# 2noise/ChatTTS

Measured on NVIDIA H100. Metric: speech-tokens/sec (GPT decode loop, 4-codebook tokens; RTF = wall / audio seconds @ 24 kHz), higher is better.
Workload: dtype f32

## Files before the change

### chattts_b200/csrc/flow.cuh

```cuda
#pragma once
#include "gpt_kernels.cuh"
#include "tc_common.cuh"

namespace ctb {

constexpr int FL_THREADS = 256;
constexpr int FL_LAUNCH_THREADS = FL_THREADS;
constexpr int FL_WARPS = 8;
constexpr int FL_SLOTS = 4;
constexpr int FL_SLOT_BYTES = 6144;
constexpr int FL_SLOT_FLOATS = FL_SLOT_BYTES / 4;
constexpr int FL_RING_BYTES = FL_WARPS * FL_SLOTS * FL_SLOT_BYTES;
constexpr int FL_SMAX = 6;
constexpr int FL_CH = 64;
constexpr int FL_PW = 66;
constexpr int FL_BMAX = 4;
constexpr int FL_ROWS = 6;
constexpr int FL_GU = 3;
constexpr int FL_QR = 2;
constexpr int FL_HEADS = 12;
constexpr int FL_RMAX = 16;

constexpr int FL_A_X = 0;
constexpr int FL_A_XO = FL_A_X + FL_BMAX * KC;
constexpr int FL_A_ACT = FL_A_XO + FL_BMAX * KC;
constexpr int FL_A_P = FL_A_ACT + FL_BMAX * 4 * KC;
constexpr int FL_A_END = FL_A_P + FL_BMAX * FL_HEADS * FL_SMAX * FL_PW;
constexpr int FL_REP_STRIDE = ((FL_A_END + 1023) / 1024) * 1024;
constexpr int FL_A_Q = 0, FL_A_KN = FL_BMAX * KC, FL_A_VN = 2 * FL_BMAX * KC;
constexpr int FL_QKV_WORDS = 3 * FL_BMAX * KC;
constexpr int FL_SROWS = 16, FL_VPAD = 1024;
constexpr int FL_A_LOGITS = FL_QKV_WORDS, FL_A_IDX = FL_A_LOGITS + FL_SROWS * FL_VPAD;
constexpr int FL_TAIL_WORDS = FL_A_IDX + 64;
constexpr size_t FL_PARITY_WORDS = (size_t)FL_RMAX * FL_REP_STRIDE + FL_TAIL_WORDS;
constexpr size_t FL_ARENA_WORDS = 2 * FL_PARITY_WORDS;
constexpr unsigned FL_EPOCH_STEP = 256;
constexpr int FL_TR_EV = 4096, FL_TR_EVN = 32, FL_TR_WORDS = FL_TR_EV + 192 * FL_TR_EVN;

enum FlowTagKind { FT_X = 0, FT_QKV = 1, FT_P = 2, FT_XO = 3, FT_ACT = 4, FT_LOGITS = 5, FT_IDX = 6 };
enum FlowStage { FS_Q0 = 0, FS_Q1 = 1, FS_KV = 2, FS_O = 3, FS_GU0 = 4, FS_GU1 = 5, FS_GU2 = 6, FS_D0 = 7, FS_D1 = 8, FS_NLAYER = 9 };

__device__ __forceinline__ void fl_bar() { asm volatile("bar.sync 1, 256;" ::: "memory"); }

struct FlowP {
  const float* W;
  int64_t layer0, layer_stride, o_wqkv, o_wo, o_wgu, o_wd, o_ln1, o_ln2, o_final_norm, o_head, o_emb_code, o_emb_text,
      o_cos, o_sin;
  int L, I, Hq, hd;
  float eps, scaling;
  float *logits, *kv;
  size_t kv_layer_floats;
  const int* block_table; int pages_per_row;
  int* seq_len;
  LoopState* st;
  int decode, col, T0, sample;
  const float* emb; const uint8_t* mask; const int32_t* ids_out;
  int max_new, num_vq, num_audio, infer_text, B;
  float* hidden_out; int hidden_stride, rows_per_item, V;
  unsigned long long* arena;
  unsigned* epoch;
  int R;
  int l2_ahead;
  unsigned long long* trace;
  int nsteps;
  int ink;
  ctb_sampler_config samp;
  const float* q_noise;
  uint8_t* finish;
  int* end_idx;
  int32_t* ids_w;
};

__device__ __forceinline__ void ll_st(unsigned long long* p, float v, uint32_t tag) {
  const unsigned long long x = ((unsigned long long)tag << 32) | (unsigned long long)__float_as_uint(v);
  asm volatile("st.relaxed.gpu.global.u64 [%0], %1;" ::"l"(p), "l"(x) : "memory");
}
__device__ __forceinline__ unsigned long long ll_ld(const unsigned long long* p) {
  unsigned long long x;
  asm volatile("ld.global.cg.u64 %0, [%1];" : "=l"(x) : "l"(p) : "memory");
  return x;
}
__device__ __forceinline__ void ll_ld2(const unsigned long long* p, unsigned long long& a, unsigned long long& b) {
  asm volatile("ld.global.cg.v2.u64 {%0,%1}, [%2];" : "=l"(a), "=l"(b) : "l"(p) : "memory");
}
__device__ __forceinline__ uint32_t ll_tag(unsigned long long x) { return (uint32_t)(x >> 32); }
__device__ __forceinline__ float ll_val(unsigned long long x) { return __uint_as_float((uint32_t)x); }

struct FlowWd {
  int* err;
  int dead;
  int spins;
};
__device__ __forceinline__ bool fl_giveup(FlowWd& wd, int code) {
  if (wd.dead) return true;
  if (++wd.spins < (1 << 20)) {
// ... 118 lines not shown
      const int bytes = e.z & 0xffff, ncopy = (e.z >> 16) & 0xf, kind = e.z >> 20;
      const float* src = (kind ? p.kv + (size_t)it.l * p.kv_layer_floats : p.W + p.layer0 + (int64_t)it.l * p.layer_stride) + e.x;
      fl_expect(bar, (uint32_t)(bytes * ncopy));
#pragma unroll
      for (int k = 0; k < 4; ++k)
        if (k < ncopy) fl_bulk(dst + k * bytes, src + (int64_t)k * e.y, (uint32_t)bytes, bar, kind ? pol_kv : pol_w);
      if (p.l2_ahead && kind == 0) {
        const float* nsrc = it.l + 1 < p.L ? src + p.layer_stride : src - (int64_t)(p.L - 1) * p.layer_stride;
#pragma unroll
        for (int k = 0; k < 4; ++k)
          if (k < ncopy)
            asm volatile("cp.async.bulk.prefetch.L2.global [%0], %1;" ::"l"(nsrc + (int64_t)k * e.y), "r"((uint32_t)bytes) : "memory");
      }
    }
    if (++it.k == it.ntab) { it.k = 0; it.l++; }
    it.n++;
    return true;
  }
  if (gs->cta * FL_WARPS + w + it.hsub * gs->NW < gs->nheads_tasks) {
    fl_issue_heads(p, gs, w, it.hsub, dst, bar, pol_w);
    it.hsub++;
    it.n++;
    return true;
  }
  return false;
}

struct FlowW {
  float* base;
  uint32_t ring;
  uint32_t bars;
  int n;
  int owed;
  FlowIss it;
  const int4* tab;
  const FlowGeo* gs;
  uint64_t pol_w, pol_kv;
};
__device__ __forceinline__ void fl_refill(const FlowP& p, FlowW& w) {
  if (w.owed > 0) {
    __syncwarp();
    fl_issue(p, w.gs, w.tab, w.it, (int)(threadIdx.x >> 5), w.ring, w.bars, w.pol_w, w.pol_kv);
    w.owed--;
  }
}
__device__ __forceinline__ const float* fl_ring_slot_at(const FlowW& w, int k) { return w.base + ((w.n + k) % FL_SLOTS) * FL_SLOT_FLOATS; }
__device__ __forceinline__ bool fl_ring_peek_n(const FlowP& p, FlowW& w, int cnt) {
  while (w.owed > FL_SLOTS - cnt) fl_refill(p, w);
  bool ok = true;
#pragma unroll
  for (int k = 0; k < 3; ++k)
    if (k < cnt) { const int n = w.n + k; ok = fl_try_wait(w.bars + (n % FL_SLOTS) * 8, (uint32_t)(n / FL_SLOTS) & 1u) && ok; }
  return ok;
}
__device__ __forceinline__ void fl_ring_wait_n(const FlowP& p, FlowW& w, int cnt, FlowWd& wd) {
  while (w.owed > FL_SLOTS - cnt) fl_refill(p, w);
  uint32_t bar[3], par[3];
#pragma unroll
  for (int k = 0; k < 3; ++k) {
    const int n = w.n + k;
    bar[k] = w.bars + (n % FL_SLOTS) * 8;
    par[k] = (uint32_t)(n / FL_SLOTS) & 1u;
  }
  wd.spins = 0;
  while (true) {
    bool ok[3];
#pragma unroll
    for (int k = 0; k < 3; ++k) ok[k] = k < cnt ? fl_try_wait(bar[k], par[k]) : true;
    if (ok[0] && ok[1] && ok[2]) break;
    if (__any_sync(0xffffffffu, fl_giveup(wd, 0x120))) { wd.dead = 1; break; }
  }
}
__device__ __forceinline__ const float* fl_ring_wait(const FlowP& p, FlowW& w, FlowWd& wd) {
  fl_ring_wait_n(p, w, 1, wd);
  return fl_ring_slot_at(w, 0);
}
__device__ __forceinline__ void fl_ring_release(const FlowP& p, FlowW& w) { w.n++; w.owed++; fl_refill(p, w); }
__device__ __forceinline__ void fl_refill_all(const FlowP& p, FlowW& w) {
  while (w.owed > 0) fl_refill(p, w);
}

template <int BT>
__device__ __forceinline__ void fl_stage768(const FlowP& p, const unsigned long long* src, uint32_t tag, float* xs, FlowWd& wd, FlowW& fw) {
  const int tid = threadIdx.x;
  unsigned long long v[BT][3];
  wd.spins = 0;
  while (true) {
    bool ok = true;
#pragma unroll
    for (int b = 0; b < BT; ++b)
      if (b < p.B) {
#pragma unroll
        for (int k = 0; k < 3; ++k) v[b][k] = ll_ld(src + b * KC + tid + 256 * k);
      }
#pragma unroll
    for (int b = 0; b < BT; ++b)
      if (b < p.B) {
#pragma unroll
        for (int k = 0; k < 3; ++k) ok = ok && (ll_tag(v[b][k]) == tag);
      }
    if (__all_sync(0xffffffffu, ok)) break;
    if (__any_sync(0xffffffffu, fl_giveup(wd, 0x200 + (tag & 0xff)))) { wd.dead = 1; break; }
  }
#pragma unroll
  for (int b = 0; b < BT; ++b) {
#pragma unroll
    for (int k = 0; k < 3; ++k) xs[b * KC + tid + 256 * k] = b < p.B ? ll_val(v[b][k]) : 0.f;
  }
  fl_bar();
}

template <int BT>
// ... 425 lines not shown
  __shared__ __align__(8) uint64_t s_nwbar[2];
  __shared__ int s_pos[BT], s_active[BT], s_page[BT];
  __shared__ float s_cos[BT * 64], s_sin[BT * 64];
  __shared__ float s_red[FL_ROWS][FL_WARPS][BT];
  __shared__ float s_resd[FL_ROWS * BT];
  __shared__ float s_am[FL_WARPS], s_al[FL_WARPS];
  __shared__ __align__(16) float s_ao[FL_WARPS][64];
  __shared__ FlowGeo s_geo;
  __shared__ __align__(16) float s_nw1[KC], s_nw2[KC];
  __shared__ int4 s_tab[FL_WARPS][FL_TMAX];
  __shared__ FlowSamp s_samp_store[BT <= 2 ? 1 : 0 + (BT > 2)];
  FlowSamp& s_samp = s_samp_store[0];

  const int tid = threadIdx.x, lane = tid & 31, warp = tid >> 5;
  constexpr int LPB = 32 / BT;
  if (tid < FL_WARPS * FL_SLOTS) mbar_init(&s_bar[tid], 1);
  if (tid < 2) mbar_init(&s_nwbar[tid], 1);
  asm volatile("fence.mbarrier_init.release.cluster;" ::: "memory");
  __syncthreads();
  pdl_trigger();
  pdl_wait();
  if (p.decode && ldg_cg(&p.st->all_finished)) return;

  constexpr bool INK = BT <= 2;
  __shared__ int s_ids[BT * 8];
  __shared__ int s_fin[BT], s_end[BT];
  __shared__ int s_allfin;
  FlowWd wd{&p.st->err, 0, 0};
  uint32_t base = (uint32_t)ldg_cg(reinterpret_cast<const int*>(p.epoch));
  int tr = 0;
#define FL_TRACE() do { if (p.trace && blockIdx.x == 0 && tid == 0 && tr < 250) p.trace[tr++] = globaltimer_ns(); } while (0)
#define FL_EV(k) do { if (p.trace && l == 10 && tid == 0) p.trace[FL_TR_EV + blockIdx.x * FL_TR_EVN + (k)] = globaltimer_ns(); } while (0)
#define FL_CK(k) do { if (p.trace && l == 10 && tid == 0 && blockIdx.x == 0) p.trace[3000 + (k)] = (unsigned long long)clock64(); } while (0)

  int ngen = p.decode ? ldg_cg(&p.st->n_gen) : 0;
  int lstep = p.decode ? ldg_cg(&p.st->step) : 0;
  if (tid < BT) {
    int act = 0, pos = 0;
    if (tid < p.B) {
      pos = ldg_cg(&p.seq_len[tid]);
      act = p.decode ? 1 : (p.mask[(size_t)tid * p.T0 + p.col] != 0);
    }
    s_pos[tid] = pos; s_active[tid] = act;
    s_fin[tid] = (tid < p.B && p.ink) ? (int)p.finish[tid] : 0;
    s_end[tid] = (tid < p.B && p.ink) ? ldg_cg(&p.end_idx[tid]) : 0;
  }
  const bool ink = INK && p.ink != 0;
  const int nrows_s = p.B * p.rows_per_item;
  const int R = p.R;
  uint64_t pol_w, pol_kv;
  asm volatile("createpolicy.fractional.L2::evict_first.b64 %0, 1.0;" : "=l"(pol_w));
  asm volatile("createpolicy.fractional.L2::evict_normal.b64 %0, 1.0;" : "=l"(pol_kv));
  int nw1_cnt = 0, nw2_cnt = 0;
  FlowW fw;
  fw.base = reinterpret_cast<float*>(fl_smem) + (size_t)warp * FL_SLOTS * FL_SLOT_FLOATS;
  fw.ring = smem_u32(fw.base);
  fw.bars = smem_u32(&s_bar[warp * FL_SLOTS]);
  fw.n = 0; fw.owed = 0;
  fw.it = FlowIss{0, 0, 0, 0, 0};
  fw.tab = s_tab[warp]; fw.gs = &s_geo; fw.pol_w = pol_w; fw.pol_kv = pol_kv;
  FlowGeo g;
  g.G = gridDim.x; g.NW = g.G * FL_WARPS; g.cta = blockIdx.x; g.warp = warp; g.lane = lane; g.gw = g.cta * FL_WARPS + warp;
  g.S = max(1, min(FL_SMAX, g.G / (p.Hq * p.B)));
  g.nheads_tasks = p.sample ? (p.rows_per_item * p.V + 1) / 2 : 0;
  const int myrep = g.cta % R;
  const int o_row = g.cta + g.G * warp;
  unsigned long long* tailw = p.arena + (size_t)FL_RMAX * FL_REP_STRIDE;
  fl_bar();

  int nwin = 0;
  if constexpr (INK) {
    if (ink && g.cta < nrows_s) {
      const int item = g.cta / p.rows_per_item, qi = g.cta % p.rows_per_item;
      const bool pen = p.samp.penalty_on && g.cta < p.samp.penalty_max_ids;
      nwin = pen ? min(ngen, p.samp.past_window) : 0;
      if (tid < nwin) s_samp.win[tid] = ldg_cg(&p.ids_out[((size_t)item * p.max_new + (ngen - nwin + tid)) * p.num_vq + qi]);
    }
  }

#define FL_PREP_STEP()                                                                                                  \
  do {                                                                                                                  \
    if (tid < BT) s_page[tid] = tid < p.B ? __ldg(p.block_table + tid * p.pages_per_row + s_pos[tid] / kPageTokens) : 0; \
    {                                                                                                                   \
      const int u = g.cta;                                                                                              \
      g.u_on = 0; g.u_b = 0; g.u_h = 0; g.u_split = 0; g.u_n = 0; g.u_nchunk = 0;                                       \
      if (u < p.B * p.Hq * g.S) {                                                                                       \
        g.u_split = u % g.S; g.u_h = (u / g.S) % p.Hq; g.u_b = u / (g.S * p.Hq);                                        \
        g.u_n = s_pos[g.u_b] + 1;                                                                                       \
        g.u_nchunk = (g.u_n + FL_CH - 1) / FL_CH;                                                                       \
        g.u_on = s_active[g.u_b] && g.u_split < min(g.u_nchunk, g.S);                                                   \
      }                                                                                                                 \
    }                                                                                                                   \
    if (tid == 0) s_geo = g;                                                                                            \
    fl_bar();                                                                                                           \
    fw.it.l = 0; fw.it.k = 0; fw.it.hsub = 0; fw.owed = 0;                                                              \
    fw.it.ntab = fl_build_table(p, &s_geo, s_tab[warp]);                                                                \
    __syncwarp();                                                                                                       \
    for (int k_ = 0; k_ < FL_SLOTS; ++k_) fl_issue(p, fw.gs, fw.tab, fw.it, warp, fw.ring, fw.bars, pol_w, pol_kv);     \
    for (int i = tid; i < BT * 64; i += FL_THREADS) {                                                                   \
      const int b = i / 64;                                                                                             \
      s_cos[i] = b < p.B ? __ldg(p.W + p.o_cos + (size_t)s_pos[b] * 64 + (i % 64)) : 0.f;                               \
      s_sin[i] = b < p.B ? __ldg(p.W + p.o_sin + (size_t)s_pos[b] * 64 + (i % 64)) : 0.f;                               \
    }                                                                                                                   \
  } while (0)

  FL_PREP_STEP();
  FL_TRACE();
#pragma unroll 1
  for (int sidx = 0;; ++sidx) {
  FL_TRACE();
  fl_nw_fetch(s_nw1, p.W + p.layer0 + p.o_ln1, &s_nwbar[0], pol_w);
  fl_nw_fetch(s_nw2, p.W + p.layer0 + p.o_ln2, &s_nwbar[1], pol_w);
  {
    float ev[BT * 3][8];
#pragma unroll
    for (int it_ = 0; it_ < BT * 3; ++it_) {
      const int i = tid + it_ * FL_THREADS, b = i / KC, k = i % KC;
#pragma unroll
      for (int q = 0; q < 8; ++q) ev[it_][q] = 0.f;
      if (b < p.B) {
        if (!p.decode) {
          ev[it_][0] = s_active[b] ? p.emb[((size_t)b * p.T0 + p.col) * KC + k] : 0.f;
        } else if (p.infer_text) {
          const int id0 = ldg_cg(p.ids_out + ((size_t)b * p.max_new + (ngen - 1)) * p.num_vq);
          ev[it_][0] = p.W[p.o_emb_text + (size_t)id0 * KC + k];
        } else {
#pragma unroll
          for (int q = 0; q < 8; ++q)
            if (q < p.num_vq) {
              const int id = sidx > 0 ? s_ids[b * 8 + q] : ldg_cg(p.ids_out + ((size_t)b * p.max_new + (ngen - 1)) * p.num_vq + q);
              ev[it_][q] = p.W[p.o_emb_code + ((size_t)q * p.num_audio + id) * KC + k];
            }
        }
      }
    }
#pragma unroll
    for (int it_ = 0; it_ < BT * 3; ++it_) {
      float v = 0.f;
#pragma unroll
      for (int q = 0; q < 8; ++q) v += ev[it_][q];
      xs[tid + it_ * FL_THREADS] = v;
    }
  }
  fl_bar();
  FL_TRACE();

  for (int l = 0; l < p.L; ++l) {
    const float* Wl = p.W + p.layer0 + (int64_t)l * p.layer_stride;
    unsigned long long* par = p.arena + (size_t)(l & 1) * FL_PARITY_WORDS;
    unsigned long long* parn = p.arena + (size_t)((l + 1) & 1) * FL_PARITY_WORDS;
    unsigned long long* qkvw = par + (size_t)FL_RMAX * FL_REP_STRIDE;
    const unsigned long long* myr = par + (size_t)myrep * FL_REP_STRIDE;
    const uint32_t tagl = base + 8u * (uint32_t)l;

    {
      float4 nw[6];
      FL_EV(0);
      fl_nw_wait(&s_nwbar[0], nw1_cnt, wd);
      const bool q_rdy = fl_ring_peek_n(p, fw, 1);
      if (l > 0) fl_stage768<BT>(p, myr + FL_A_X, tagl + FT_X, xs, wd, fw);
      else fl_bar();
      FL_EV(1);
      fl_refill_all(p, fw);
      fl_load_nw_s(s_nw1, nw, lane);
      float x[BT][24];
      fl_load_x<BT>(xs, x, lane);
      float res_o = 0.f;
      if (fl_o_valid(g)) res_o = xs[(lane / LPB) * KC + o_row];
      fl_norm<BT>(x, nw, p.eps);
      float res_keep = res_o;
#pragma unroll 1
      for (int j = 0; j < FL_QR; ++j) {
        if (!fl_q_valid(g, j)) continue;
        if (!(j == 0 && q_rdy)) fl_ring_wait_n(p, fw, 1, wd);
        const float* slot = fl_ring_slot_at(fw, 0);
        FL_EV(2);
        float a0[BT], a1[BT];
        fl_dot2<BT>(slot, x, a0, a1, lane);
        warp_reduce_scatter<BT>(a0);
        warp_reduce_scatter<BT>(a1);
        const int b = lane / LPB;
        if ((lane % LPB) == 0 && b < p.B && s_active[b]) {
          const int half = p.hd / 2, nq = p.Hq * half;
          int t = g.gw + j * g.NW, which = 0;
          if (t >= 2 * nq) { which = 2; t -= 2 * nq; }
          else if (t >= nq) { which = 1; t -= nq; }
          const int h = t / half, jj = t % half;
          const float v0 = a0[0], v1 = a1[0];
          float o0 = v0, o1 = v1;
          if (which < 2) {
            const float* cs = s_cos + b * 64;
            const float* sn = s_sin + b * 64;
            o0 = __fadd_rn(__fmul_rn(v0, cs[jj]), __fmul_rn(-v1, sn[jj]));
            o1 = __fadd_rn(__fmul_rn(v1, cs[jj + half]), __fmul_rn(v0, sn[jj + half]));
          }
          unsigned long long* dst = qkvw + (which == 0 ? FL_A_Q : which == 1 ? FL_A_KN : FL_A_VN) + b * KC + h * 64;
// ... 19 lines not shown
          int chunk;
          if (!fl_kv_more(g, sb, chunk)) break;
          const bool have = fl_kv_valid(g, chunk);
          const float* slot = have ? fl_ring_wait(p, fw, wd) : nullptr;
          const int tbase = chunk * FL_CH + warp * 8 + grp;
          float4 k0[2], k1[2], v0[2], v1[2];
#pragma unroll
          for (int i = 0; i < 2; ++i) {
            const int t = tbase + 4 * i;
            k0[i] = k1[i] = v0[i] = v1[i] = make_float4(0.f, 0.f, 0.f, 0.f);
            if (have && t < pos) {
              const float* kr = slot + (grp + 4 * i) * 64 + sub * 8;
              const float* vr = kr + 8 * 64;
              k0[i] = *reinterpret_cast<const float4*>(kr); k1[i] = *reinterpret_cast<const float4*>(kr + 4);
              v0[i] = *reinterpret_cast<const float4*>(vr); v1[i] = *reinterpret_cast<const float4*>(vr + 4);
            }
          }
          if (sb == 0) {
            const unsigned long long* qp = qkvw + FL_A_Q + b * KC + h * 64 + sub * 8;
            unsigned long long w[8];
            wd.spins = 0;
            while (true) {
              bool ok = true;
#pragma unroll
              for (int k = 0; k < 4; ++k) ll_ld2(qp + 2 * k, w[2 * k], w[2 * k + 1]);
#pragma unroll
              for (int k = 0; k < 8; ++k) ok = ok && (ll_tag(w[k]) == tagl + FT_QKV);
              if (__all_sync(0xffffffffu, ok)) break;
              if (__any_sync(0xffffffffu, fl_giveup(wd, 0x300))) { wd.dead = 1; break; }
            }
#pragma unroll
            for (int k = 0; k < 8; ++k) q[k] = ll_val(w[k]);
          }
          if (sb == 0) { FL_EV(4); fl_refill_all(p, fw); }
          {
            const bool mine0 = (tbase == pos), mine1 = (tbase + 4 == pos);
            if (__any_sync(0xffffffffu, mine0 || mine1)) {
              const unsigned long long* kp = qkvw + FL_A_KN + b * KC + h * 64 + sub * 8;
              const unsigned long long* vp = qkvw + FL_A_VN + b * KC + h * 64 + sub * 8;
              unsigned long long kw[8], vw[8];
              wd.spins = 0;
              while (true) {
                bool ok = true;
                if (mine0 || mine1) {
#pragma unroll
                  for (int k = 0; k < 4; ++k) { ll_ld2(kp + 2 * k, kw[2 * k], kw[2 * k + 1]); ll_ld2(vp + 2 * k, vw[2 * k], vw[2 * k + 1]); }
#pragma unroll
                  for (int k = 0; k < 8; ++k) ok = ok && (ll_tag(kw[k]) == tagl + FT_QKV) && (ll_tag(vw[k]) == tagl + FT_QKV);
                }
                if (__all_sync(0xffffffffu, ok)) break;
                if (__any_sync(0xffffffffu, fl_giveup(wd, 0x301))) { wd.dead = 1; break; }
              }
              if (mine0 || mine1) {
                const int i = mine0 ? 0 : 1;
                const float4 a = make_float4(ll_val(kw[0]), ll_val(kw[1]), ll_val(kw[2]), ll_val(kw[3]));
                const float4 bq = make_float4(ll_val(kw[4]), ll_val(kw[5]), ll_val(kw[6]), ll_val(kw[7]));
                const float4 cq = make_float4(ll_val(vw[0]), ll_val(vw[1]), ll_val(vw[2]), ll_val(vw[3]));
                const float4 dq = make_float4(ll_val(vw[4]), ll_val(vw[5]), ll_val(vw[6]), ll_val(vw[7]));
                if (i == 0) { k0[0] = a; k1[0] = bq; v0[0] = cq; v1[0] = dq; }
                else { k0[1] = a; k1[1] = bq; v0[1] = cq; v1[1] = dq; }
              }
            }
          }
          float sc[2], m = -INFINITY;
#pragma unroll
          for (int i = 0; i < 2; ++i) {
            float s = q[0] * k0[i].x + q[1] * k0[i].y + q[2] * k0[i].z + q[3] * k0[i].w + q[4] * k1[i].x + q[5] * k1[i].y +
// ... 31 lines not shown
          }
          fl_bar();
          if (lane < 8) {
            *reinterpret_cast<float4*>(&s_ao[warp][lane * 8]) = make_float4(o[0], o[1], o[2], o[3]);
            *reinterpret_cast<float4*>(&s_ao[warp][lane * 8 + 4]) = make_float4(o[4], o[5], o[6], o[7]);
            if (lane == 0) { s_am[warp] = m; s_al[warp] = lsum; }
          }
          fl_bar();
          if (tid < 64) {
            float cm = M;
#pragma unroll
            for (int w = 0; w < FL_WARPS; ++w) cm = fmaxf(cm, s_am[w]);
            const float fo = (M > -INFINITY) ? expf(M - cm) : 0.f;
            L *= fo; O *= fo;
#pragma unroll
            for (int w = 0; w < FL_WARPS; ++w) {
              const float f = (s_am[w] > -INFINITY) ? expf(s_am[w] - cm) : 0.f;
              L = fmaf(f, s_al[w], L);
              O = fmaf(f, s_ao[w][tid], O);
            }
            M = cm;
          }
        }
        FL_EV(14);
        if (tid < 64) {
          unsigned long long* P = par + FL_A_P + ((size_t)(b * FL_HEADS + h) * FL_SMAX + g.u_split) * FL_PW;
          for (int r = 0; r < R; ++r) {
            unsigned long long* Pr = P + (size_t)r * FL_REP_STRIDE;
            ll_st(Pr + tid, O, tagl + FT_P);
            if (tid == 0) { ll_st(Pr + 64, M, tagl + FT_P); ll_st(Pr + 65, L, tagl + FT_P); }
          }
        }
        FL_EV(15);
        if (pend_kv) fl_ring_release(p, fw);
      }
      FL_TRACE();
      FL_EV(5);

      fl_bar();
      if (l + 1 < p.L || p.sample) fl_nw_fetch(s_nw1, l + 1 < p.L ? Wl + p.layer_stride + p.o_ln1 : p.W + p.o_final_norm, &s_nwbar[0], pol_w);
      const bool o_rdy = fl_o_valid(g) ? fl_ring_peek_n(p, fw, 1) : true;
      fl_stage_attn<BT>(p, myr + FL_A_P, tagl + FT_P, xs, wd, g.S, s_pos, s_active);
      fl_refill_all(p, fw);
      FL_EV(6);
      if (fl_o_valid(g)) {
        fl_load_x<BT>(xs, x, lane);
        if (!o_rdy) fl_ring_wait_n(p, fw, 1, wd);
        const float* slot = fl_ring_slot_at(fw, 0);
        FL_EV(7);
        float a0[BT];
        fl_dot1<BT>(slot, x, a0, lane);
        warp_reduce_scatter<BT>(a0);
        const float out = __fadd_rn(res_keep, a0[0]);
        fl_bcast_store<BT>(par, R, FL_A_XO + (size_t)(lane / LPB) * KC + o_row, out, tagl + FT_XO, p.B, lane);
        fl_ring_release(p, fw);
      }
      FL_TRACE();
      FL_EV(8);
    }

    {
      float4 nw[6];
      fl_nw_wait(&s_nwbar[1], nw2_cnt, wd);
      int ngu = 0;
#pragma unroll
      for (int j = 0; j < FL_GU; ++j) ngu += fl_gu_valid(g, j, p.I) ? 1 : 0;
      const bool gu_rdy = fl_ring_peek_n(p, fw, ngu);
      fl_bar();
      FL_CK(8);
      fl_stage768<BT>(p, myr + FL_A_XO, tagl + FT_XO, xs, wd, fw);
      fl_refill_all(p, fw);
      fl_load_nw_s(s_nw2, nw, lane);
      FL_EV(9);
      FL_CK(9);
      if (tid < FL_ROWS * BT) {
        const int b = tid % BT, j = tid / BT, row = g.cta + g.G * j;
        s_resd[tid] = row < KC ? xs[b * KC + row] : 0.f;
      }
      float x[BT][24];
      fl_load_x<BT>(xs, x, lane);
      FL_CK(10);
      fl_norm<BT>(x, nw, p.eps);
      FL_CK(11);
      {
        FL_CK(0);
        const float4* sl[FL_GU];
#pragma unroll
        for (int j = 0; j < FL_GU; ++j) sl[j] = reinterpret_cast<const float4*>(fl_ring_slot_at(fw, j)) + lane;
        if (!gu_rdy) fl_ring_wait_n(p, fw, ngu, wd);
        FL_EV(16);
        FL_CK(1);
        float acc[8 * BT];
#pragma unroll
        for (int k = 0; k < 8 * BT; ++k) acc[k] = 0.f;
#pragma unroll
        for (int i = 0; i < 6; ++i) {
#pragma unroll
          for (int j = 0; j < FL_GU; ++j)
            if (j < ngu) {
              const float4 u = sl[j][i * 32], v = sl[j][KC / 4 + i * 32];
#pragma unroll
              for (int b = 0; b < BT; ++b) {
                float& a0 = acc[(2 * j) * BT + b];
                float& a1 = acc[(2 * j + 1) * BT + b];
                a0 = fmaf(u.x, x[b][4 * i], a0); a0 = fmaf(u.y, x[b][4 * i + 1], a0);
                a0 = fmaf(u.z, x[b][4 * i + 2], a0); a0 = fmaf(u.w, x[b][4 * i + 3], a0);
                a1 = fmaf(v.x, x[b][4 * i], a1); a1 = fmaf(v.y, x[b][4 * i + 1], a1);
                a1 = fmaf(v.z, x[b][4 * i + 2], a1); a1 = fmaf(v.w, x[b][4 * i + 3], a1);
              }
            }
        }
        FL_CK(2);
        warp_reduce_scatter<8 * BT>(acc);
        FL_CK(3);
        constexpr int LPV = 32 / (8 * BT);
        const int gl = lane & 7, b = (gl / LPV) % BT, base8 = lane & ~7;
        const float gv = __shfl_sync(0xffffffffu, acc[0], base8 + b * LPV);
        const float uv = __shfl_sync(0xffffffffu, acc[0], base8 + BT * LPV + b * LPV);
        if ((lane >> 3) < ngu && b < p.B) {
          const float sg = __fdiv_rn(gv, __fadd_rn(1.0f, expf(-gv)));
          const float act = __fmul_rn(sg, uv);
          unsigned long long* d = par + FL_A_ACT + (size_t)b * p.I + (g.gw + (lane >> 3) * g.NW);
          for (int rr = (gl % LPV) + (gl >= BT * LPV ? LPV : 0); rr < R; rr += 2 * LPV) ll_st(d + (size_t)rr * FL_REP_STRIDE, act, tagl + FT_ACT);
        }
        FL_CK(5);
        for (int j = 0; j < ngu; ++j) fl_ring_release(p, fw);
        FL_CK(6);
      }
      FL_TRACE();
      FL_EV(10);
    }

    {
      float xd[BT][12];
      const int nr0_ = fl_d_rows(g, 0, 4), nr1_ = fl_d_rows(g, 4, FL_ROWS);
      const bool d_rdy = fl_ring_peek_n(p, fw, nr1_ > 0 ? 2 : 1);
      {
        const int kslice = p.I / FL_WARPS;
#pragma unroll
        for (int b = 0; b < BT; ++b) {
#pragma unroll
          for (int k = 0; k < 12; ++k) xd[b][k] = 0.f;
          if (b < p.B) {
            const unsigned long long* ap = myr + FL_A_ACT + (size_t)b * p.I + warp * kslice;
            unsigned long long w[12];
            wd.spins = 0;
            bool sentinel_ok = false;
            int it_s = 0, it_f = 0;
            if (b == 0) FL_CK(12);
            while (true) {
              ++it_s;
              ll_ld2(ap + lane * 4, w[0], w[1]);
              if (sentinel_ok || __all_sync(0xffffffffu, ll_tag(w[0]) == tagl + FT_ACT && ll_tag(w[1]) == tagl + FT_ACT)) {
                if (!sentinel_ok && b == 0) FL_CK(13);
                sentinel_ok = true;
                ++it_f;
                bool ok = ll_tag(w[0]) == tagl + FT_ACT && ll_tag(w[1]) == tagl + FT_ACT;
                ll_ld2(ap + lane * 4 + 2, w[2], w[3]);
#pragma unroll
                for (int i = 1; i < 3; ++i) {
                  ll_ld2(ap + (i * 32 + lane) * 4, w[4 * i], w[4 * i + 1]);
                  ll_ld2(ap + (i * 32 + lane) * 4 + 2, w[4 * i + 2], w[4 * i + 3]);
                }
#pragma unroll
                for (int k = 2; k < 12; ++k) ok = ok && (ll_tag(w[k]) == tagl + FT_ACT);
                if (__all_sync(0xffffffffu, ok)) break;
              }
              if (__any_sync(0xffffffffu, fl_giveup(wd, 0x500))) { wd.dead = 1; break; }
            }
            if (b == 0) { FL_CK(14); if (p.trace && l == 10 && tid == 0 && blockIdx.x == 0) { p.trace[3015] = it_s; p.trace[3016] = it_f; } }
#pragma unroll
            for (int k = 0; k < 12; ++k) xd[b][k] = ll_val(w[k]);
          }
        }
      }
      FL_EV(11);
      fl_refill_all(p, fw);
      int e_tasks = 0;
      {
        const int nr0 = nr0_, nr1 = nr1_;
        const float* s0 = fl_ring_slot_at(fw, 0);
        const float* s1 = nr1 > 0 ? fl_ring_slot_at(fw, 1) : s0;
        if (!d_rdy) fl_ring_wait_n(p, fw, nr1 > 0 ? 2 : 1, wd);
        FL_EV(17);
        float acc[8 * BT];
#pragma unroll
        for (int k = 0; k < 8 * BT; ++k) acc[k] = 0.f;
#pragma unroll
        for (int i = 0; i < 3; ++i) {
#pragma unroll
          for (int k = 0; k < FL_ROWS; ++k) {
            const bool valid = k < 4 ? (k < nr0) : (k - 4 < nr1);
            if (valid) {
              const float4 u = (reinterpret_cast<const float4*>((k < 4 ? s0 : s1) + (k & 3) * (3072 / FL_WARPS)) + lane)[i * 32];
#pragma unroll
              for (int b = 0; b < BT; ++b) {
                float& a = acc[k * BT + b];
                a = fmaf(u.x, xd[b][4 * i], a); a = fmaf(u.y, xd[b][4 * i + 1], a);
                a = fmaf(u.z, xd[b][4 * i + 2], a); a = fmaf(u.w, xd[b][4 * i + 3], a);
              }
            }
          }
        }
        warp_reduce_scatter<8 * BT>(acc);
        constexpr int LPV = 32 / (8 * BT);
        const int vi = lane / LPV, k = vi / BT, b = vi % BT;
        if ((lane % LPV) == 0 && k < FL_ROWS) s_red[k][warp][b] = acc[0];
        e_tasks = nr1 > 0 ? 2 : 1;
      }
      FL_EV(12);
      fl_bar();
      if (l + 1 < p.L) fl_nw_fetch(s_nw2, Wl + p.layer_stride + p.o_ln2, &s_nwbar[1], pol_w);
      if (tid < FL_ROWS * BT * 8) {
        const int e = tid >> 3, b = e % BT, j = e / BT, row = g.cta + g.G * j;
        if (row < KC && b < p.B) {
          float v = s_red[j][0][b];
#pragma unroll
          for (int w = 1; w < FL_WARPS; ++w) v = __fadd_rn(v, s_red[j][w][b]);
          const float out = __fadd_rn(s_resd[e], v);
          for (int r = tid & 7; r < R; r += 8)
            ll_st(parn + (size_t)r * FL_REP_STRIDE + FL_A_X + (size_t)b * KC + row, out, tagl + 8u + FT_X);
        }
      }
      for (int k = 0; k < e_tasks; ++k) fl_ring_release(p, fw);
      FL_TRACE();
      FL_EV(13);
    }
  }

  if (p.sample) {
    const unsigned long long* myr = p.arena + (size_t)(p.L & 1) * FL_PARITY_WORDS + (size_t)myrep * FL_REP_STRIDE;
    float4 nw[6];
    fl_nw_wait(&s_nwbar[0], nw1_cnt, wd);
    fl_bar();
    fl_stage768<BT>(p, myr + FL_A_X, base + 8u * (uint32_t)p.L + FT_X, xs, wd, fw);
    fl_refill_all(p, fw);
    fl_load_nw_s(s_nw1, nw, lane);
    float x[BT][24];
    fl_load_x<BT>(xs, x, lane);
    fl_norm<BT>(x, nw, p.eps);
    if (p.hidden_out != nullptr && blockIdx.x == 0 && warp == 0) {
#pragma unroll
      for (int b = 0; b < BT; ++b)
        if (b < p.B) {
          float4* dst = reinterpret_cast<float4*>(p.hidden_out + (size_t)b * p.hidden_stride + (size_t)ngen * KC);
#pragma unroll
          for (int i = 0; i < 6; ++i) dst[i * 32 + lane] = make_float4(x[b][4 * i], x[b][4 * i + 1], x[b][4 * i + 2], x[b][4 * i + 3]);
        }
    }
    const int nrows = p.rows_per_item * p.V;
    const uint32_t tagh = base + 8u * (uint32_t)p.L + FT_LOGITS;
    for (int j = 0; fl_h_valid(g, j); ++j) {
      const int t = g.gw + j * g.NW;
      const float* slot = fl_ring_wait(p, fw, wd);
      float a0[BT], a1[BT];
      fl_dot2<BT>(slot, x, a0, a1, lane);
      warp_reduce_scatter<BT>(a0);
      warp_reduce_scatter<BT>(a1);
      const int b = lane / LPB;
      if ((lane % LPB) == 0 && b < p.B) {
        const int r0 = 2 * t, q0 = r0 / p.V, c0 = r0 % p.V;
        const int q1 = (r0 + 1) / p.V, c1 = (r0 + 1) % p.V;
        if (ink) {
          ll_st(tailw + FL_A_LOGITS + (size_t)(b * p.rows_per_item + q0) * FL_VPAD + c0, a0[0], tagh);
          if (r0 + 1 < nrows) ll_st(tailw + FL_A_LOGITS + (size_t)(b * p.rows_per_item + q1) * FL_VPAD + c1, a1[0], tagh);
        } else {
          p.logits[((size_t)b * p.rows_per_item + q0) * p.V + c0] = a0[0];
          if (r0 + 1 < nrows) p.logits[((size_t)b * p.rows_per_item + q1) * p.V + c1] = a1[0];
        }
// ... 69 lines not shown
        s_allfin = !notall;
        if (blockIdx.x == 0) {
          if (!notall) p.st->all_finished = 1;
          p.st->n_gen = ngen + 1;
          p.st->step = lstep + 1;
        }
      }
      fl_bar();
      FL_TRACE();
    }
  }
  ngen++; lstep++;
  base += FL_EPOCH_STEP;
  if (!more || s_allfin) {
    if (more) {
      const int outst = fw.it.n - fw.n;
      for (int k = 0; k < outst; ++k) {
        const int n = fw.n + k;
        wd.spins = 0;
        while (!fl_try_wait(fw.bars + (n % FL_SLOTS) * 8, (uint32_t)(n / FL_SLOTS) & 1u))
          if (__any_sync(0xffffffffu, fl_giveup(wd, 0x700))) { wd.dead = 1; break; }
      }
    }
    break;
  }
  }
  if (blockIdx.x == 0) {
    if (tid < p.B) p.seq_len[tid] = s_pos[tid];
    if (tid == 0) *p.epoch = base;
  }
#undef FL_TRACE
#undef FL_EV
#undef FL_CK
#undef FL_PREP_STEP
}

}
```

### chattts_b200/csrc/gpt_api.cu

```cuda
#include <stdarg.h>

#include <map>
#include <mutex>
#include <vector>

#include <cudaTypedefs.h>

#define CTB_GPT_KERNELS_IMPL
#include "gpt_kernels.cuh"
#include "tc_decode.cuh"
#include "mega.cuh"
#include "flow.cuh"
#include "prefill.cuh"
#include "tc_gemm.cuh"
#include "kv_pool.cuh"

namespace ctb {

thread_local char g_err[512] = {0};
std::atomic<uint64_t> g_launches{0};

int set_err(int code, const char* fmt, ...) {
  va_list ap;
  va_start(ap, fmt);
// ... 32 lines not shown
  float *x, *qbuf, *attn, *mlp, *logits, *kv, *part;
  int *block_table, *seq_len, *pos, *counter, *end_idx;
  int32_t* idx;
  uint8_t *active, *finish;
  LoopState* st;
  size_t kv_layer_elems;
  size_t kv_bytes;
  int bt_B; size_t bt_per_row;
  int B, T0, max_new, infer_text, started;
  ctb_sampler_config sampler;
  const float* q_noise;
  const float* emb;
  const uint8_t* mask;
  int32_t* ids_out;
  float* hiddens_out;
  cudaGraphExec_t graph_exec;
  uint64_t graph_kernels;
  cudaStream_t cap_stream;
  bool use_tc, tc_ready;
  int tc_min_batch;
  bool pf_enabled;
  float *gw_hi, *gw_lo;
  float *pf_resid, *pf_xn, *pf_qkv, *pf_q, *pf_attn, *pf_gu, *pf_h, *pf_ones, *pf_zeros;
  int *pf_npre, *pf_nvalid;
  uint8_t* pf_mask;
  size_t pf_rows;
  bool mega_ok;
  int mega_max_batch;
  unsigned* bar;
  unsigned long long* trace;
  bool flow_ok;
  int flow_R;
  int flow_l2_ahead;
  int flow_max_batch;
  unsigned long long* flow_arena;
  unsigned* flow_epoch;
  int steps_enqueued;
  float *tc_wqkv, *tc_wgu, *tc_heads_code, *tc_heads_text;
  float *x_hi, *x_lo, *attn_hi, *attn_lo, *h_hi, *h_lo;
  int tc_rows;
  CUtensorMap *m_wqkv, *m_wo, *m_wgu, *m_wd;
  CUtensorMap m_hcode, m_htext;
  CUtensorMap m_x[3][2], m_attn[3][2], m_h[3][2];
  bool use_graph;
  int engine;
  int phase;
  RowState* rows;
  ctb_sampler_config* cfgs;
  float* eng_noise;
  int* eng_slot;
  float* eng_text_logits;
  int32_t* eng_text_idx;
  int eng_text;
  cudaGraphExec_t graph_exec_text;
  uint64_t graph_kernels_text;
  float* eng_logprobs;
  int eng_served;
  std::vector<SlotRecord> slot;
  int prec;
  bool tc_base;
  __half *w16_qkv, *w16_wo, *w16_gu, *w16_wd;
  CUtensorMap *m16_wqkv, *m16_wo, *m16_wgu, *m16_wd;
  float* gw16;
  float* pf_wzero;
  int pg_pages;
  bool pg_poison;
// ... 357 lines not shown
  h->bpad_max = ((c->max_batch + bt - 1) / bt) * bt;
  const size_t Bp = h->bpad_max, d = c->hidden_size;
  const size_t nq = (size_t)c->num_heads * c->head_dim;
  int rc;
#define TRY(e) if ((rc = (e)) != CTB_OK) { ctb_gpt_destroy(h); return rc; }
  TRY(dalloc(&h->x, Bp * d));
  TRY(dalloc(&h->qbuf, Bp * nq));
  TRY(dalloc(&h->attn, Bp * nq));
  TRY(dalloc(&h->mlp, Bp * c->intermediate_size));
  const size_t nlog = std::max((size_t)c->num_vq * c->num_audio_tokens, (size_t)c->num_text_tokens);
  TRY(dalloc(&h->logits, Bp * nlog));
  h->kv = nullptr; h->kv_layer_elems = 0; h->kv_bytes = 0;
  TRY(dalloc(&h->part, (size_t)c->max_batch * c->num_heads * h->nsplit_max * (c->head_dim + 2)));
  TRY(dalloc(&h->block_table, (size_t)c->max_batch * h->pages_per_row));
  TRY(dalloc(&h->seq_len, Bp));
  TRY(dalloc(&h->pos, Bp));
  TRY(dalloc(&h->counter, (size_t)c->max_batch * c->num_heads));
  TRY(dalloc(&h->end_idx, Bp));
  TRY(dalloc(&h->idx, Bp * c->num_vq));
  TRY(dalloc(&h->active, Bp));
  TRY(dalloc(&h->finish, Bp));
  TRY(dalloc(&h->st, 1));
  TRY(dalloc(&h->bar, 4));
  if (getenv("CTB_MEGA_TRACE")) TRY(dalloc(&h->trace, FL_TR_WORDS));
  h->flow_ok = getenv("CTB_NO_FLOW") == nullptr && g_num_sms >= 128 && g_num_sms <= 191 && c->intermediate_size == 4 * KC &&
               c->num_heads == c->num_kv_heads && c->num_heads * c->head_dim == KC && c->num_heads <= FL_HEADS;
  if (h->flow_ok) {
    TRY(dalloc(&h->flow_arena, FL_ARENA_WORDS));
    TRY(dalloc(&h->flow_epoch, 4));
    const unsigned e0 = FL_EPOCH_STEP;
    cudaMemcpy(h->flow_epoch, &e0, sizeof(e0), cudaMemcpyHostToDevice);
    h->flow_R = getenv("CTB_FLOW_R") ? std::max(1, std::min(FL_RMAX, atoi(getenv("CTB_FLOW_R")))) : 1;
    h->flow_l2_ahead = getenv("CTB_FLOW_L2_AHEAD") ? atoi(getenv("CTB_FLOW_L2_AHEAD")) : 0;
    h->flow_max_batch = getenv("CTB_FLOW_MAX_BATCH") ? std::max(0, std::min(FL_BMAX, atoi(getenv("CTB_FLOW_MAX_BATCH")))) : 1;
  }
#undef TRY
  h->use_graph = getenv("CTB_NO_GRAPH") == nullptr;
  h->pf_enabled = getenv("CTB_NO_BATCHED_PREFILL") == nullptr;
  h->mega_ok = getenv("CTB_NO_MEGA") == nullptr && g_num_sms >= 128 && c->intermediate_size == 4 * KC &&
               (c->hidden_size / 2 + g_num_sms - 1) / g_num_sms <= MG_DOWN_PAIRS;
  h->mega_max_batch = getenv("CTB_MEGA_MAX_BATCH") ? std::min(8, atoi(getenv("CTB_MEGA_MAX_BATCH"))) : 4;
  constexpr int kTcMinBatch = 9;
  h->tc_ready = getenv("CTB_GPT_FMA") == nullptr && c->max_batch <= 32 &&
                (getenv("CTB_GPT_TC") != nullptr || c->max_batch >= kTcMinBatch);
  h->tc_min_batch = getenv("CTB_GPT_TC") != nullptr ? 1 : kTcMinBatch;
  if (h->tc_ready && (rc = tc_setup(h)) != CTB_OK) { ctb_gpt_destroy(h); return rc; }
  *out = h;
  return CTB_OK;
}

extern "C" int ctb_gpt_destroy(ctb_gpt* h) {
  if (!h) return CTB_OK;
  if (h->graph_exec) cudaGraphExecDestroy(h->graph_exec);
  if (h->graph_exec_text) cudaGraphExecDestroy(h->graph_exec_text);
  if (h->cap_stream) cudaStreamDestroy(h->cap_stream);
  void* ptrs[] = {h->x, h->qbuf, h->attn, h->mlp, h->logits, h->kv, h->part, h->block_table, h->seq_len,
                  h->pos, h->counter, h->end_idx, h->idx, h->active, h->finish, h->st, h->tc_wqkv, h->tc_wgu,
                  h->tc_heads_code, h->tc_heads_text, h->x_hi, h->x_lo, h->attn_hi, h->attn_lo, h->h_hi, h->h_lo, h->bar, h->trace, h->flow_arena, h->flow_epoch, h->gw_hi, h->gw_lo, h->pf_resid, h->pf_xn, h->pf_qkv, h->pf_q,
                  h->pf_attn, h->pf_gu, h->pf_h, h->pf_ones, h->pf_zeros, h->pf_npre, h->pf_nvalid,
                  h->pf_mask, h->rows, h->cfgs, h->eng_noise, h->eng_slot, h->eng_text_logits, h->eng_text_idx,
                  h->pg_stage};
  delete[] h->m_wqkv; delete[] h->m_wo; delete[] h->m_wgu; delete[] h->m_wd;
  for (void* p : ptrs) if (p) cudaFree(p);
  fp16_free(h);
  delete h;
  return CTB_OK;
// ... 338 lines not shown
  { int rc = ensure_smem_attr((const void*)k_flow<BT>, (int)smem); if (rc) return rc; }
  cudaLaunchConfig_t cfg{};
  cfg.gridDim = dim3(g_num_sms); cfg.blockDim = dim3(FL_LAUNCH_THREADS); cfg.dynamicSmemBytes = smem; cfg.stream = s;
  cudaLaunchAttribute attr[1];
  attr[0].id = cudaLaunchAttributeCooperative;
  attr[0].val.cooperative = 1;
  cfg.attrs = attr; cfg.numAttrs = 1;
  CTB_CUDA(cudaLaunchKernelEx(&cfg, k_flow<BT>, fp));
  CTB_LAUNCH_CHECK();
  return CTB_OK;
}

static bool flow_ink(const ctb_gpt* h);

static int launch_step_flow(ctb_gpt* h, int col, bool sample, cudaStream_t s, int nsteps = 0) {
  const ctb_gpt_config& c = h->cfg;
  const ctb_gpt_layout& L = h->lay;
  FlowP m{};
  m.W = h->W; m.layer0 = L.layer0; m.layer_stride = L.layer_stride; m.o_wqkv = L.wqkv; m.o_wo = L.wo; m.o_wgu = L.wgate_up;
  m.o_wd = L.wdown; m.o_ln1 = L.ln1; m.o_ln2 = L.ln2; m.o_final_norm = L.final_norm;
  m.o_head = h->infer_text ? L.head_text : L.head_code; m.o_emb_code = L.emb_code; m.o_emb_text = L.emb_text;
  m.o_cos = L.rope_cos; m.o_sin = L.rope_sin;
  m.L = c.num_layers; m.I = c.intermediate_size; m.Hq = c.num_heads; m.hd = c.head_dim; m.eps = c.rms_eps;
  m.scaling = 1.0f / sqrtf((float)c.head_dim);
  m.logits = h->logits; m.kv = h->kv; m.kv_layer_floats = h->kv_layer_elems; m.block_table = h->block_table;
  m.pages_per_row = h->pages_per_row; m.seq_len = h->seq_len; m.st = h->st;
  m.decode = col < 0; m.col = col < 0 ? 0 : col; m.T0 = h->T0; m.sample = sample ? 1 : 0;
  m.emb = h->emb; m.mask = h->mask; m.ids_out = h->ids_out; m.max_new = h->max_new; m.num_vq = c.num_vq;
  m.num_audio = c.num_audio_tokens; m.infer_text = h->infer_text; m.B = h->B;
  m.hidden_out = h->hiddens_out; m.hidden_stride = h->max_new * c.hidden_size;
  m.rows_per_item = h->infer_text ? 1 : c.num_vq; m.V = h->infer_text ? c.num_text_tokens : c.num_audio_tokens;
  m.arena = h->flow_arena; m.epoch = h->flow_epoch; m.R = h->flow_R; m.trace = h->trace;
  m.l2_ahead = h->flow_l2_ahead;
  m.ink = nsteps > 0 ? 1 : 0; m.nsteps = nsteps > 0 ? nsteps : 1; m.samp = h->sampler; m.q_noise = h->q_noise;
  m.finish = h->finish; m.end_idx = h->end_idx; m.ids_w = h->ids_out;
  switch (bt_for(h->B)) {
    case 1: return launch_step_flow_t<1>(m, s);
    case 2: return launch_step_flow_t<2>(m, s);
    default: return launch_step_flow_t<4>(m, s);
  }
}

static bool use_flow(const ctb_gpt* h) { return h->flow_ok && !h->engine && !h->use_tc && h->B <= h->flow_max_batch; }
static bool flow_ink(const ctb_gpt* h) {
  static const bool off = getenv("CTB_FLOW_NO_INK") != nullptr;
  return !off && use_flow(h) && !h->infer_text && h->B <= 2 && h->cfg.num_audio_tokens <= FL_VPAD &&
         h->B * h->cfg.num_vq <= FL_SROWS && h->cfg.num_vq <= 8;
}

static int launch_finalize(ctb_gpt* h, cudaStream_t s) {
  const ctb_gpt_config& c = h->cfg;
  FinalP fp{};
  fp.st = h->st; fp.B = h->B; fp.rows_per_item = h->infer_text ? 1 : c.num_vq; fp.num_vq = c.num_vq;
  fp.max_new = h->max_new; fp.eos = h->sampler.eos_token; fp.idx = h->idx; fp.ids_out = h->ids_out;
  fp.finish = h->finish; fp.end_idx = h->end_idx;
  if (h->engine) {
    fp.rows = h->rows; fp.want = h->phase; fp.idx_text = h->eng_text_idx;
    CTB_CUDA(launch_pdl(k_finalize_rows, dim3(1), dim3(256), 0, s, fp));
  } else {
    CTB_CUDA(launch_pdl(k_finalize, dim3(1), dim3(256), 0, s, fp));
  }
  CTB_LAUNCH_CHECK();
  return CTB_OK;
}

static int enqueue_step(ctb_gpt* h, int col, bool sample, cudaStream_t s) {
// ... 1044 lines not shown
```

Measured before the change: 2256.

## Pace weight-ring refills after gate-up and down stages to defer prefetch issue

```diff
diff --git a/chattts_b200/csrc/flow.cuh b/chattts_b200/csrc/flow.cuh
--- a/chattts_b200/csrc/flow.cuh
+++ b/chattts_b200/csrc/flow.cuh
@@ -36,6 +36,9 @@
 constexpr size_t FL_ARENA_WORDS = 2 * FL_PARITY_WORDS;
 constexpr unsigned FL_EPOCH_STEP = 256;
 constexpr int FL_TR_EV = 4096, FL_TR_EVN = 32, FL_TR_WORDS = FL_TR_EV + 192 * FL_TR_EVN;
+
+constexpr int FL_EV_ACT_REL = 18, FL_EV_X_REL = 20, FL_EV_PB = 22;
+enum FlowPbWindow { FPB_X = 0, FPB_QKV = 1, FPB_P = 2, FPB_XO = 3, FPB_ACT = 4, FL_PB_WINDOWS = 5 };
 
 enum FlowTagKind { FT_X = 0, FT_QKV = 1, FT_P = 2, FT_XO = 3, FT_ACT = 4, FT_LOGITS = 5, FT_IDX = 6 };
 enum FlowStage { FS_Q0 = 0, FS_Q1 = 1, FS_KV = 2, FS_O = 3, FS_GU0 = 4, FS_GU1 = 5, FS_GU2 = 6, FS_D0 = 7, FS_D1 = 8, FS_NLAYER = 9 };
@@ -61,6 +64,7 @@
   unsigned* epoch;
   int R;
   int l2_ahead;
+  int pace;
   unsigned long long* trace;
   int nsteps;
   int ink;
@@ -245,6 +249,7 @@
   uint32_t bars;
   int n;
   int owed;
+  int defer;
   FlowIss it;
   const int4* tab;
   const FlowGeo* gs;
@@ -288,9 +293,25 @@
   fl_ring_wait_n(p, w, 1, wd);
   return fl_ring_slot_at(w, 0);
 }
+constexpr int FL_PACE_ACT = 2;
+constexpr int FL_PACE_X = 1;
 __device__ __forceinline__ void fl_ring_release(const FlowP& p, FlowW& w) { w.n++; w.owed++; fl_refill(p, w); }
 __device__ __forceinline__ void fl_refill_all(const FlowP& p, FlowW& w) {
   while (w.owed > 0) fl_refill(p, w);
+}
+__device__ __forceinline__ void fl_ring_release_paced(const FlowP& p, FlowW& w, int cnt, int k) {
+#pragma unroll 1
+  for (int j = 0; j < cnt; ++j) {
+    if (j < k) fl_ring_release(p, w);
+    else { w.n++; w.defer++; }
+  }
+}
+__device__ __forceinline__ void fl_post_deferred(const FlowP& p, FlowW& w) {
+#pragma unroll 1
+  for (; w.defer > 0; --w.defer) {
+    __syncwarp();
+    fl_issue(p, w.gs, w.tab, w.it, (int)(threadIdx.x >> 5), w.ring, w.bars, w.pol_w, w.pol_kv);
+  }
 }
 
 template <int BT>
@@ -782,6 +803,9 @@
 #define FL_TRACE() do { if (p.trace && blockIdx.x == 0 && tid == 0 && tr < 250) p.trace[tr++] = globaltimer_ns(); } while (0)
 #define FL_EV(k) do { if (p.trace && l == 10 && tid == 0) p.trace[FL_TR_EV + blockIdx.x * FL_TR_EVN + (k)] = globaltimer_ns(); } while (0)
 #define FL_CK(k) do { if (p.trace && l == 10 && tid == 0 && blockIdx.x == 0) p.trace[3000 + (k)] = (unsigned long long)clock64(); } while (0)
+  __shared__ int s_pmark[FL_WARPS], s_pwin[FL_PB_WINDOWS];
+#define FL_PB_MARK(c) do { if (p.trace && (c) && lane == 0) s_pmark[warp] = fw.it.n; } while (0)
+#define FL_PB_ADD(c, k) do { if (p.trace && (c) && lane == 0) atomicAdd(&s_pwin[k], fw.it.n - s_pmark[warp]); } while (0)
 
   int ngen = p.decode ? ldg_cg(&p.st->n_gen) : 0;
   int lstep = p.decode ? ldg_cg(&p.st->step) : 0;
@@ -806,7 +830,7 @@
   fw.base = reinterpret_cast<float*>(fl_smem) + (size_t)warp * FL_SLOTS * FL_SLOT_FLOATS;
   fw.ring = smem_u32(fw.base);
   fw.bars = smem_u32(&s_bar[warp * FL_SLOTS]);
-  fw.n = 0; fw.owed = 0;
+  fw.n = 0; fw.owed = 0; fw.defer = 0;
   fw.it = FlowIss{0, 0, 0, 0, 0};
   fw.tab = s_tab[warp]; fw.gs = &s_geo; fw.pol_w = pol_w; fw.pol_kv = pol_kv;
   FlowGeo g;
@@ -843,7 +867,7 @@
     }                                                                                                                   \
     if (tid == 0) s_geo = g;                                                                                            \
     fl_bar();                                                                                                           \
-    fw.it.l = 0; fw.it.k = 0; fw.it.hsub = 0; fw.owed = 0;                                                              \
+    fw.it.l = 0; fw.it.k = 0; fw.it.hsub = 0; fw.owed = 0; fw.defer = 0;                                                \
     fw.it.ntab = fl_build_table(p, &s_geo, s_tab[warp]);                                                                \
     __syncwarp();                                                                                                       \
     for (int k_ = 0; k_ < FL_SLOTS; ++k_) fl_issue(p, fw.gs, fw.tab, fw.it, warp, fw.ring, fw.bars, pol_w, pol_kv);     \
@@ -905,13 +929,16 @@
 
     {
       float4 nw[6];
+      if (p.trace && l == 9 && tid < FL_PB_WINDOWS) s_pwin[tid] = 0;
       FL_EV(0);
       fl_nw_wait(&s_nwbar[0], nw1_cnt, wd);
       const bool q_rdy = fl_ring_peek_n(p, fw, 1);
       if (l > 0) fl_stage768<BT>(p, myr + FL_A_X, tagl + FT_X, xs, wd, fw);
       else fl_bar();
       FL_EV(1);
-      fl_refill_all(p, fw);
+      FL_PB_ADD(l == 10, FPB_X);
+      fl_post_deferred(p, fw);
+      FL_PB_MARK(l == 10);
       fl_load_nw_s(s_nw1, nw, lane);
       float x[BT][24];
       fl_load_x<BT>(xs, x, lane);
@@ -997,7 +1024,7 @@
 #pragma unroll
             for (int k = 0; k < 8; ++k) q[k] = ll_val(w[k]);
           }
-          if (sb == 0) { FL_EV(4); fl_refill_all(p, fw); }
+          if (sb == 0) { FL_EV(4); FL_PB_ADD(l == 10, FPB_QKV); fl_refill_all(p, fw); }
           {
             const bool mine0 = (tbase == pos), mine1 = (tbase + 4 == pos);
             if (__any_sync(0xffffffffu, mine0 || mine1)) {
@@ -1095,6 +1122,7 @@
           }
         }
         FL_EV(15);
+        FL_PB_MARK(l == 10);
         if (pend_kv) fl_ring_release(p, fw);
       }
       FL_TRACE();
@@ -1104,7 +1132,9 @@
       if (l + 1 < p.L || p.sample) fl_nw_fetch(s_nw1, l + 1 < p.L ? Wl + p.layer_stride + p.o_ln1 : p.W + p.o_final_norm, &s_nwbar[0], pol_w);
       const bool o_rdy = fl_o_valid(g) ? fl_ring_peek_n(p, fw, 1) : true;
       fl_stage_attn<BT>(p, myr + FL_A_P, tagl + FT_P, xs, wd, g.S, s_pos, s_active);
+      FL_PB_ADD(l == 10, g.u_on ? FPB_P : FPB_QKV);
       fl_refill_all(p, fw);
+      FL_PB_MARK(l == 10);
       FL_EV(6);
       if (fl_o_valid(g)) {
         fl_load_x<BT>(xs, x, lane);
@@ -1132,7 +1162,9 @@
       fl_bar();
       FL_CK(8);
       fl_stage768<BT>(p, myr + FL_A_XO, tagl + FT_XO, xs, wd, fw);
+      FL_PB_ADD(l == 10, FPB_XO);
       fl_refill_all(p, fw);
+      FL_PB_MARK(l == 10);
       fl_load_nw_s(s_nw2, nw, lane);
       FL_EV(9);
       FL_CK(9);
@@ -1187,7 +1219,9 @@
           for (int rr = (gl % LPV) + (gl >= BT * LPV ? LPV : 0); rr < R; rr += 2 * LPV) ll_st(d + (size_t)rr * FL_REP_STRIDE, act, tagl + FT_ACT);
         }
         FL_CK(5);
-        for (int j = 0; j < ngu; ++j) fl_ring_release(p, fw);
+        FL_EV(FL_EV_ACT_REL);
+        fl_ring_release_paced(p, fw, ngu, p.pace ? FL_PACE_ACT : FL_SLOTS);
+        FL_EV(FL_EV_ACT_REL + 1);
         FL_CK(6);
       }
       FL_TRACE();
@@ -1238,7 +1272,9 @@
         }
       }
       FL_EV(11);
-      fl_refill_all(p, fw);
+      FL_PB_ADD(l == 10, FPB_ACT);
+      fl_post_deferred(p, fw);
+      FL_PB_MARK(l == 9);
       int e_tasks = 0;
       {
         const int nr0 = nr0_, nr1 = nr1_;
@@ -1273,6 +1309,7 @@
       }
       FL_EV(12);
       fl_bar();
+      if (p.trace && l == 10 && tid < FL_PB_WINDOWS) p.trace[FL_TR_EV + blockIdx.x * FL_TR_EVN + FL_EV_PB + tid] = s_pwin[tid];
       if (l + 1 < p.L) fl_nw_fetch(s_nw2, Wl + p.layer_stride + p.o_ln2, &s_nwbar[1], pol_w);
       if (tid < FL_ROWS * BT * 8) {
         const int e = tid >> 3, b = e % BT, j = e / BT, row = g.cta + g.G * j;
@@ -1285,7 +1322,9 @@
             ll_st(parn + (size_t)r * FL_REP_STRIDE + FL_A_X + (size_t)b * KC + row, out, tagl + 8u + FT_X);
         }
       }
-      for (int k = 0; k < e_tasks; ++k) fl_ring_release(p, fw);
+      FL_EV(FL_EV_X_REL);
+      fl_ring_release_paced(p, fw, e_tasks, p.pace ? FL_PACE_X : FL_SLOTS);
+      FL_EV(FL_EV_X_REL + 1);
       FL_TRACE();
       FL_EV(13);
     }
@@ -1297,7 +1336,7 @@
     fl_nw_wait(&s_nwbar[0], nw1_cnt, wd);
     fl_bar();
     fl_stage768<BT>(p, myr + FL_A_X, base + 8u * (uint32_t)p.L + FT_X, xs, wd, fw);
-    fl_refill_all(p, fw);
+    fl_post_deferred(p, fw);
     fl_load_nw_s(s_nw1, nw, lane);
     float x[BT][24];
     fl_load_x<BT>(xs, x, lane);
@@ -1433,6 +1472,8 @@
 #undef FL_TRACE
 #undef FL_EV
 #undef FL_CK
+#undef FL_PB_MARK
+#undef FL_PB_ADD
 #undef FL_PREP_STEP
 }
 
diff --git a/chattts_b200/csrc/gpt_api.cu b/chattts_b200/csrc/gpt_api.cu
--- a/chattts_b200/csrc/gpt_api.cu
+++ b/chattts_b200/csrc/gpt_api.cu
@@ -88,6 +88,7 @@
   bool flow_ok;
   int flow_R;
   int flow_l2_ahead;
+  int flow_pace;
   int flow_max_batch;
   unsigned long long* flow_arena;
   unsigned* flow_epoch;
@@ -511,6 +512,7 @@
     cudaMemcpy(h->flow_epoch, &e0, sizeof(e0), cudaMemcpyHostToDevice);
     h->flow_R = getenv("CTB_FLOW_R") ? std::max(1, std::min(FL_RMAX, atoi(getenv("CTB_FLOW_R")))) : 1;
     h->flow_l2_ahead = getenv("CTB_FLOW_L2_AHEAD") ? atoi(getenv("CTB_FLOW_L2_AHEAD")) : 0;
+    h->flow_pace = getenv("CTB_FLOW_PACE") ? atoi(getenv("CTB_FLOW_PACE")) != 0 : 1;
     h->flow_max_batch = getenv("CTB_FLOW_MAX_BATCH") ? std::max(0, std::min(FL_BMAX, atoi(getenv("CTB_FLOW_MAX_BATCH")))) : 1;
   }
 #undef TRY
@@ -915,6 +917,7 @@
   m.rows_per_item = h->infer_text ? 1 : c.num_vq; m.V = h->infer_text ? c.num_text_tokens : c.num_audio_tokens;
   m.arena = h->flow_arena; m.epoch = h->flow_epoch; m.R = h->flow_R; m.trace = h->trace;
   m.l2_ahead = h->flow_l2_ahead;
+  m.pace = h->flow_pace;
   m.ink = nsteps > 0 ? 1 : 0; m.nsteps = nsteps > 0 ? nsteps : 1; m.samp = h->sampler; m.q_noise = h->q_noise;
   m.finish = h->finish; m.end_idx = h->end_idx; m.ids_w = h->ids_out;
   switch (bt_for(h->B)) {
```

New measurement: 2331 (median of 6 runs). +3.3%, better.
